# cbs228/sameold

Measured on AMD Instinct MI355X. Metric: Msamples/s demodulated (batched 22.05 kHz channels) + % HBM roofline, 1/8 GPU, higher is better.
Workload: dtype f32

## Files before the change

sameold_amd/csrc/same_batch.cpp:

```cpp
#include <hip/hip_runtime.h>

#include <algorithm>
#include <chrono>
#include <cstdio>
#include <cstdlib>
#include <cstring>
#include <deque>
#include <new>
#include <string>
#include <utility>
#include <vector>

#include "../../include/same_rx.h"
#include "same_config.h"
#include "same_device.h"
#include "same_harvest.h"
#include "same_hipmem.h"
#include "same_launch.h"
#include "same_resets.h"
#include "same_transport.h"

using same::fail;

namespace {
// ... 19 lines not shown
    hipStream_t last_stream = nullptr;
    same::DevBuf<float4> d_taps;
    same::DevBuf<void> d_state_blob;
    struct Slot {
        same::DevBuf<same::DevEvent> d_events;
        uint32_t event_cap() const { return (uint32_t)d_events.size(); }
        same::DevBuf<uint32_t> d_sort;
        same::PinnedBuf<uint32_t> h_sort;
        same::DevBuf<same::DevEvent> d_sorted;
        uint32_t sort_bins = 0;
        same::DevBuf<uint8_t> d_bursts;
        uint32_t burst_cap() const { return (uint32_t)(d_bursts.size() / same::kBurstCap); }
        same::DevBuf<uint32_t> d_counters;
        same::MappedBuf<uint32_t> h_counters;
        same::Event ev_start, ev_stop, ev_done, ev_planned;
        same::Event ev_k0, ev_k1;
        bool have_k = false;
        bool timed = false;
        same::PinnedBuf<void> h_events, h_bursts;
        bool in_flight = false;
        uint64_t seq = 0;
        uint64_t end_counter = 0;
        bool chunked = false;
        same::ChunkGeom geom{};
        uint64_t end_blocks = 0;
        same::DevBuf<uint64_t> d_handover;
        same::PinnedBuf<uint64_t> h_handover;
        bool per_channel = false;
        same::DevBuf<uint32_t> d_geom;
        same::PinnedBuf<uint32_t> h_geom;
        same::CoherentBuf<uint32_t> h_reset;
        same::CoherentBuf<uint32_t> h_counts;
        same::PinnedBuf<uint64_t> h_wake_up;
        bool dev_transport = false;
        same::CoherentBuf<same::DevMessage> h_near;
        uint32_t near_cap() const { return (uint32_t)h_near.size(); }
        same::DevBuf<same::DevMessage> d_msgs;
        uint32_t msg_cap() const { return (uint32_t)d_msgs.size(); }
        same::PinnedBuf<void> h_msgs;
        bool captured = false;
        same::DevBuf<same::cap::Span> d_spans;
        uint32_t span_cap() const { return (uint32_t)d_spans.size(); }
        same::DevBuf<float> d_pool;
        same::DevBuf<same::cap::Cursors> d_cap_cur;
        same::MappedBuf<same::cap::Cursors> h_cap_cur;
        same::PinnedBuf<void> h_spans, h_pool;
    } slot[2];
    struct TimePar {
        bool enabled = false;
        uint32_t max_chunks = 0, min_own = 0, warmup = 0;
        uint32_t cap_columns = 0;
        uint32_t carved_columns = 0;
        int carved_family = -1;
        same::Params Pv{};
        same::State Sv{};
        same::DevBuf<void> blob;
        same::DevBuf<void> blob_fresh;
        size_t fresh_bytes = 0;
        same::DevBuf<same::StateArrayDesc> d_desc_in, d_desc_out;
        uint32_t n_desc = 0;
        same::DevBuf<uint32_t> d_final_col;
        same::DevBuf<float> d_energy;
        same::DevBuf<float> d_hist;
        same::Event ev_plan_prev; bool plan_recorded = false;
        int knob_plan_stream = 0;
        int sort_mode = -1;
        uint32_t last_chunks = 1;
        bool last_per_channel = false;
        same::Family family = same::Family::kPipe;
        int knob_prologue = 0;
    } tp;
    uint64_t launch_seq = 0;
    hipStream_t copy_stream = nullptr;
    struct Windowed {
        bool on = false;
        uint32_t window = 0;
        uint32_t fill = 0;
        same::DevBuf<void> d_buf;
        same::Event ev_buf;
        hipStream_t buf_stream = nullptr; bool buf_used = false;
        same::Event ev_read[2];
        uint64_t n_reads = 0;
        hipStream_t read_stream = nullptr;
    } inv;
    hipStream_t plan_stream = nullptr;
    float last_ms = 0.0f;
    bool overflowed = false;
    std::string record_path;
    bool kernel_fault = false;
    same::Request want;
    same::Mode mode;
    same::Choice plain;
    same::Params Pfm{};
    same::Family last_family = same::Family::kGeneric;
    bool sym_launched = false;
    bool debug = false;
    same::DevBuf<void> d_stage, d_stage2;
    same::DevBuf<void> d_upload;
    same::DevBuf<void> d_zero;
    same::Event ev_order;
    bool timing = false;
    bool have_timing = false;
    float last_demod_ms = 0.0f;
    same::PinnedBuf<uint64_t> h_wake;
    bool wake_ordered = false;
    std::vector<uint32_t> ragged_by;
    bool messages_only = false;
    bool dev_transport = false;
    bool last_dev_transport = false;
    same::DevBuf<void> d_thot, d_tcold;
    same::ResetLedger resets;
    std::vector<uint32_t> reset_list, reset_now, reset_cols;
    same::EventLog events;
    same::Replay replay{resets, events};
    struct Audio {
// ... 79 lines not shown
    rx->P.knob_pipe_split = tri("SAME_PIPE_SPLIT");
#ifdef SAME_PROFILE
    rx->P.knob_mirror = tri("SAME_MIRROR");
    rx->P.knob_pipe_share = tri("SAME_PIPE_SHARE");
    rx->P.knob_prio = num("SAME_PIPE_PRIO", 0);
#endif
    rx->P.knob_fast_dense = tri("SAME_FAST_DENSE");
    rx->P.knob_sym = tri("SAME_SYM");
    rx->want.sym_max_channels = (uint32_t)std::max(0, num("SAME_SYM_MAX", 1 << 30));
    rx->debug = rx->replay.debug = std::getenv("SAME_DEBUG") != nullptr;
    { const char *e = std::getenv("SAME_RECORD_HARVEST"); rx->record_path = e ? e : ""; }
    rx->replay.host_threads = std::max(0, num("SAME_HOST_THREADS", 0));
    rx->tp.sort_mode = num("SAME_TP_SORT", -1);
    rx->tp.knob_plan_stream = tri("SAME_TP_PLAN_STREAM");
    rx->tp.knob_prologue = tri("SAME_TP_PROLOGUE");
    rx->want.knob_relaxed = tri("SAME_RELAXED");
    { const char *e = std::getenv("SAME_RELAXED_KERNEL"); rx->P.knob_relaxed_kernel = !e ? 0 : (std::strcmp(e, "solo") == 0 ? 1 : (std::strcmp(e, "duo") == 0 ? 2 : 0)); }
    { const char *e = std::getenv("SAME_TP_KERNEL"); rx->want.knob_tp_kernel = !e ? 0 : (std::strcmp(e, "wave") == 0 ? 2 : (std::strcmp(e, "pipe") == 0 ? 1 : 0)); }
}

int ensure_output(same_batch *rx, same_batch::Slot &sl, size_t n_samples, same::Output &O, size_t n_columns = 0)
{
    const size_t n_ch = n_columns ? n_columns : rx->P.n_channels;
    const double symbols = (double)n_samples * 520.83 / (double)rx->P.input_rate;
    const size_t per_chan_events = (size_t)(symbols / 8.0) + 16;
    const size_t per_chan_bursts = (size_t)(symbols / 160.0) + 4;
    size_t ecap = std::min<size_t>(per_chan_events * n_ch, 0x7fffffffu / sizeof(same::DevEvent));
    size_t bcap = std::min<size_t>(per_chan_bursts * n_ch, 0x7fffffffu / same::kBurstCap);
    HIP_TRY(sl.d_events.ensure(ecap));
    HIP_TRY(sl.d_bursts.ensure(bcap * same::kBurstCap));
// ... 5 lines not shown
    }
    HIP_TRY(sl.d_sorted.ensure(sl.d_events.size()));
    HIP_TRY(sl.d_sort.ensure(2 * n_ch + 1 + same::event_sort_extra_words((uint32_t)n_ch)));
    HIP_TRY(sl.h_sort.ensure(n_ch + 1));
    sl.sort_bins = (uint32_t)n_ch;
    O.events = sl.d_events; O.event_cap = sl.event_cap();
    O.bursts = sl.d_bursts; O.burst_cap = sl.burst_cap();
    O.n_events = sl.d_counters; O.n_bursts = sl.d_counters + 1; O.overflow = sl.d_counters + 2;
    return SAME_OK;
}

template <typename SampleT>
hipError_t launch_family(same::Family f, const same::Params &P, const same::State &S, const same::Output &O, const float4 *taps, const SampleT *x,
                         uint32_t n_blocks, uint64_t counter0, hipStream_t stream, const same::PipeChunks &pc = same::PipeChunks{})
{
    switch (f) {
    case same::Family::kSym: return same::launch_demod_sym(P, S, O, taps, x, n_blocks, counter0, stream, pc);
    case same::Family::kPipeFastmath: return same::launch_demod_pipe(P, S, O, taps, x, n_blocks, counter0, stream, pc, true);
    case same::Family::kPipe: return same::launch_demod_pipe(P, S, O, taps, x, n_blocks, counter0, stream, pc, false);
    case same::Family::kWaveRelaxed: return same::launch_demod_relaxed(P, S, O, taps, x, n_blocks, counter0, stream, pc);
    case same::Family::kFast: return same::launch_demod_fast(P, S, O, taps, x, n_blocks, counter0, stream);
    case same::Family::kGeneric: break;
    }
    return hipErrorInvalidValue;
}

void reset_channel_host(same_batch *rx, uint32_t c, uint64_t pos)
{
    rx->replay.reset_channel(c, pos);
    if (rx->h_wake) rx->h_wake[c] = 0;
// ... 97 lines not shown
    const int oi = (int)(&other - rx->slot);
    for (uint32_t c = 0; c < C; ++c) {
        const uint64_t w = rx->h_wake[c];
        sl.h_wake_up[c] = w && other.in_flight ? w + rx->resets.pending_shift(oi, c) : w;
    }
    if (other.in_flight) {
        HIP_TRY(hipMemcpyAsync(rx->S.wake_sample, sl.h_wake_up, (size_t)C * sizeof(uint64_t), hipMemcpyHostToDevice, rx->last_stream));
        HIP_TRY(hipEventRecord(other.ev_done, rx->last_stream));
    } else {
        HIP_TRY(hipMemcpyAsync(rx->S.wake_sample, sl.h_wake_up, (size_t)C * sizeof(uint64_t), hipMemcpyHostToDevice, rx->copy_stream));
        HIP_TRY(hipStreamSynchronize(rx->copy_stream));
    }
    return SAME_OK;
}

int harvest_slot(same_batch *rx, same_batch::Slot &sl)
{
    if (!sl.in_flight) return SAME_OK;
    const bool dbg = rx->debug;
    auto t_begin = std::chrono::steady_clock::now();
    HIP_TRY(hipEventSynchronize(sl.ev_done));
    sl.in_flight = false;
    if (sl.timed) {
        HIP_TRY(hipEventElapsedTime(&rx->last_ms, sl.ev_start, sl.ev_stop));
        rx->last_demod_ms = rx->last_ms;
        if (sl.have_k) HIP_TRY(hipEventElapsedTime(&rx->last_demod_ms, sl.ev_k0, sl.ev_k1));
        rx->have_timing = true;
    }
    auto t_waited = std::chrono::steady_clock::now();
    const uint32_t n_events = std::min(sl.h_counters[0], sl.event_cap());
    if (dbg)
        std::fprintf(stderr, "[same] harvest: %u device events (%u bursts), cap %u/%u\n", sl.h_counters[0],
                     sl.h_counters[1], sl.event_cap(), sl.burst_cap());
    const uint32_t n_bursts = std::min(sl.h_counters[1], sl.burst_cap());
    if (sl.h_counters[2] & (3u | same::kMessageLogOverflow)) rx->overflowed = true;
    if (sl.h_counters[2] & 4u) rx->kernel_fault = true;
    if (sl.dev_transport) return harvest_messages(rx, sl, t_begin, t_waited);
    const size_t ev_bytes = (size_t)n_events * sizeof(same::DevEvent), bu_bytes = (size_t)n_bursts * same::kBurstCap;
    HIP_TRY(grow_pinned(sl.h_events, ev_bytes));
    HIP_TRY(grow_pinned(sl.h_bursts, bu_bytes));
    const uint32_t n_ch = rx->P.n_channels;
    const uint32_t n_bins = sl.chunked ? sl.geom.n_chunks * n_ch : n_ch;
    if (n_bins != sl.sort_bins) return fail(SAME_EINVAL, "internal: event sort made for %u columns, launch has %u", sl.sort_bins, n_bins);
    HIP_TRY(hipMemcpyAsync(sl.h_sort, sl.d_sort + n_bins, ((size_t)n_bins + 1) * sizeof(uint32_t), hipMemcpyDeviceToHost, rx->copy_stream));
    if (n_events) HIP_TRY(hipMemcpyAsync(sl.h_events, sl.d_sorted, ev_bytes, hipMemcpyDeviceToHost, rx->copy_stream));
    HIP_TRY(hipStreamSynchronize(rx->copy_stream));
    if (n_bursts) HIP_TRY(hipMemcpyAsync(sl.h_bursts, sl.d_bursts, bu_bytes, hipMemcpyDeviceToHost, rx->copy_stream));
    if (sl.chunked) {
        HIP_TRY(hipMemcpyAsync(sl.h_handover, sl.d_handover, (size_t)n_bins * sizeof(uint64_t), hipMemcpyDeviceToHost, rx->copy_stream));
        if (sl.per_channel)
            HIP_TRY(hipMemcpyAsync(sl.h_geom, sl.d_geom, (size_t)2 * n_bins * sizeof(uint32_t), hipMemcpyDeviceToHost, rx->copy_stream));
    }
    if (n_bursts || sl.chunked) HIP_TRY(hipStreamSynchronize(rx->copy_stream));
    auto t_copied = std::chrono::steady_clock::now();
    const same::HarvestInput in{sl.h_sort, static_cast<same::DevEvent *>(sl.h_events.get()), static_cast<const uint8_t *>(sl.h_bursts.get()),
                                sl.h_handover, sl.h_geom};
    if (!rx->record_path.empty()) { const int rrc = record_harvest(rx, sl, in, n_events, n_bursts, rx->record_path.c_str()); if (rrc != SAME_OK) return rrc; }
    std::vector<uint32_t> rearm;
    same::HarvestTimes times;
    same::HarvestLaunch launch;
    launch.chunked = sl.chunked; launch.per_channel = sl.per_channel; launch.geom = sl.geom;
    launch.end_blocks = sl.end_blocks; launch.end_counter = sl.end_counter;
    int rc = rx->replay.replay(launch, in, n_events, n_bursts, rearm, times);
    if (rc) return rc;
    {
        const int si = (int)(&sl - rx->slot);
        const same::ResetLedger::SlotShift &sh = rx->resets.shift_due(si);
        if (!rx->replay.thot.empty())
            for (size_t i = 0; i < sh.channels.size(); ++i)
// ... 4 lines not shown
        const int si = (int)(&sl - rx->slot);
        const std::vector<uint32_t> &due = rx->resets.host_due(si);
        for (uint32_t c : due) reset_channel_host(rx, c, rx->resets.rec_pos(si));
        rx->resets.done_host(si);
    }
    if (!rearm.empty()) {
        if (!rx->h_wake) {
            HIP_TRY(rx->h_wake.ensure(rx->P.n_channels));
            std::memset(rx->h_wake, 0, (size_t)rx->P.n_channels * sizeof(uint64_t));
        }
        for (uint32_t c : rearm) rx->h_wake[c] = rx->replay.tr(c).force_eom_at();
        if (rx->wake_ordered) {
            int rc2 = upload_wake_ordered(rx, sl);
            if (rc2) return rc2;
        } else {
        HIP_TRY(hipMemcpyAsync(rx->S.wake_sample, rx->h_wake, (size_t)rx->P.n_channels * sizeof(uint64_t), hipMemcpyHostToDevice, rx->copy_stream));
        HIP_TRY(hipStreamSynchronize(rx->copy_stream));
        }
    }
    if (dbg) {
        auto t_end = std::chrono::steady_clock::now();
        auto ms = [](auto a, auto b) { return std::chrono::duration<double, std::milli>(b - a).count(); };
        std::fprintf(stderr, "[same] harvest timing: wait %.2f ms, copy %.2f ms, sort %.2f ms, replay on %u threads %.2f ms, "
                             "queue %.2f ms\n",
                     ms(t_begin, t_waited), ms(t_waited, t_copied), ms(t_copied, times.sorted), times.n_threads,
                     ms(times.sorted, times.replayed), ms(times.replayed, t_end));
    }
    return SAME_OK;
}

int harvest(same_batch *rx)
{
// ... 38 lines not shown
    HIP_TRY(sl.d_handover.ensure(columns));
    HIP_TRY(sl.h_handover.ensure(columns));
    return SAME_OK;
}

int ensure_wide_state(same_batch *rx, uint32_t columns)
{
    same_batch::TimePar &tp = rx->tp;
    if (tp.carved_columns == columns && tp.carved_family == (int)tp.family) return SAME_OK;
    int rc = harvest(rx);
    if (rc) return rc;
    HIP_TRY(hipDeviceSynchronize());
    tp.Pv = same::wide_params(rx->P, columns, same::is_fastmath(tp.family), same::tp_more_than_one_round(columns));
    if (columns > tp.cap_columns) {
        tp.cap_columns = 0;
        HIP_TRY(tp.blob.reset());
        HIP_TRY(tp.blob_fresh.reset());
        const size_t bytes = carve_state(tp.Pv, nullptr, tp.Sv);
        HIP_TRY(tp.blob.ensure(bytes));
        HIP_TRY(hipMemset(tp.blob, 0, bytes));
        HIP_TRY(tp.blob_fresh.ensure(bytes));
        tp.cap_columns = columns;
    }
    const size_t blob_bytes = carve_state(tp.Pv, (char *)tp.blob.get(), tp.Sv);
    {
        same::State Sf{};
        carve_state(tp.Pv, (char *)tp.blob_fresh.get(), Sf);
        HIP_TRY(hipMemset(tp.blob_fresh, 0, blob_bytes));
        HIP_TRY(same::launch_init_state(tp.Pv, Sf, 0, nullptr, 0));
        HIP_TRY(hipDeviceSynchronize());
        tp.fresh_bytes = (size_t)(reinterpret_cast<char *>(tp.Sv.fr_msg) - static_cast<char *>(tp.blob.get()));
    }
    std::vector<same::StateArrayDesc> in, out;
    list_state_arrays(rx->P, rx->S, tp.Sv, in);
    list_state_arrays(rx->P, tp.Sv, rx->S, out);
    tp.n_desc = (uint32_t)in.size();
    HIP_TRY(tp.d_desc_in.ensure(in.size()));
    HIP_TRY(tp.d_desc_out.ensure(out.size()));
    HIP_TRY(tp.d_final_col.ensure(rx->P.n_channels));
    HIP_TRY(hipMemcpy(tp.d_desc_in, in.data(), in.size() * sizeof(same::StateArrayDesc), hipMemcpyHostToDevice));
    HIP_TRY(hipMemcpy(tp.d_desc_out, out.data(), out.size() * sizeof(same::StateArrayDesc), hipMemcpyHostToDevice));
    tp.carved_columns = columns;
    tp.carved_family = (int)tp.family;
    return SAME_OK;
}

struct Ragged {
    const uint32_t *counts = nullptr;
    uint32_t m = 0;
    uint32_t row_off = 0;
};

struct RaggedLaunch {
    uint32_t row0 = 0;
    size_t n_lock = 0;
};


int begin_launch(same_batch *rx, same_batch::Slot &sl, const same_batch::Slot &prev, hipStream_t stream)
{
    int rc = harvest_slot(rx, sl);
    if (rc) return rc;
    if (prev.in_flight && rx->last_stream != stream) HIP_TRY(hipStreamWaitEvent(stream, prev.ev_done, 0));
    return launch_pending_resets(rx, sl, stream);
}

int begin_timing(same_batch *rx, same_batch::Slot &sl, hipStream_t stream)
{
    sl.timed = rx->timing;
    if (sl.timed) HIP_TRY(hipEventRecord(sl.ev_start, stream));
    return SAME_OK;
}

int tp_reserve(same_batch *rx, same_batch::Slot &sl, uint32_t columns, size_t n, const same::PipeChunks &pc, uint32_t block_len, same::Output &O)
{
    int rc = ensure_wide_state(rx, columns);
    if (rc) return rc;
    rc = ensure_output(rx, sl, std::min<size_t>(n, 3 * (size_t)pc.nominal_blocks * block_len + 65536), O, columns);
    if (rc) return rc;
    return ensure_handover(sl, columns);
}

int tp_start(same_batch *rx, same_batch::Slot &sl, uint32_t columns, const char *layout, hipStream_t stream, bool *sort_bins_empty)
{
    same_batch::TimePar &tp = rx->tp;
    const uint32_t C = rx->P.n_channels;
    *sort_bins_empty = false;
    if (tp.knob_prologue >= 0) {
        HIP_TRY(same::launch_tp_prologue(tp.blob, tp.blob_fresh, tp.fresh_bytes, sl.d_handover, sl.d_sort, columns, sl.d_counters, stream));
        *sort_bins_empty = sl.sort_bins == columns;
    } else {
        HIP_TRY(same::launch_counters(sl.d_counters, sl.h_counters.dev(), 0, stream));
        HIP_TRY(same::launch_init_state(tp.Pv, tp.Sv, 0, stream, C));
        HIP_TRY(same::launch_fill_u64(sl.d_handover, columns, same::kNoHandover, stream));
    }
    if (rx->debug) std::fprintf(stderr, "[same] time-parallel launch: %u columns (%s), start-up: %s\n", columns, layout,
                                tp.knob_prologue >= 0 ? "prologue kernel" : "separate launches");
    HIP_TRY(same::launch_copy_state_columns(tp.d_desc_in, tp.n_desc, C, columns, nullptr, C, stream));
    return SAME_OK;
}

int tp_hand_back(same_batch *rx, same_batch::Slot &sl, const same::ChunkGeom &geom, const uint32_t *own_start, hipStream_t stream)
{
    same_batch::TimePar &tp = rx->tp;
    const uint32_t C = rx->P.n_channels;
    if (own_start) HIP_TRY(same::launch_chunk_final_column_pc(sl.d_handover, own_start, C, geom.n_chunks, rx->counter, tp.d_final_col, stream));
    else HIP_TRY(same::launch_chunk_final_column(sl.d_handover, C, geom, tp.d_final_col, stream));
    HIP_TRY(same::launch_copy_state_columns(tp.d_desc_out, tp.n_desc, geom.n_chunks * C, C, tp.d_final_col, C, stream));
    return SAME_OK;
}

template <typename SampleT>
int demod_tail(same_batch *rx, const same::Output &O, const SampleT *rows, size_t n, uint64_t counter0, hipStream_t stream)
{
    const hipError_t e = same::launch_demod(rx->P, rx->S, O, rx->d_taps, rows, (uint32_t)n, counter0, stream);
    if (e != hipSuccess) return fail(SAME_EHIP, "demod kernel launch failed: %s", hipGetErrorString(e));
    return SAME_OK;
}
int demod_tail_corner(same_batch *rx, const same::Output &O, const float *corner, size_t pitch, size_t r, uint64_t counter0, hipStream_t stream)
{
    const uint32_t C = rx->P.n_channels;
    HIP_TRY(rx->d_stage.ensure(r * C * sizeof(float)));
    HIP_TRY(rx->d_stage2.ensure(r * C * sizeof(float)));
// ... 80 lines not shown
        bool sort_bins_empty = false;
        same::Output O{};
        if (n_chunks > 1u) {
            const uint32_t C = rx->P.n_channels, columns = n_chunks * C;
            const size_t fbk = geom.block_len;
            rc = tp_reserve(rx, sl, columns, n, pc, geom.block_len, O);
            if (rc) return rc;
            pc.handover = sl.d_handover;
            same_batch::TimePar &tp = rx->tp;
            rc = begin_timing(rx, sl, stream);
            if (rc) return rc;
            rc = tp_start(rx, sl, columns, "time-major", stream, &sort_bins_empty);
            if (rc) return rc;
            const SampleT *xp = d_x + done * C;
            const uint32_t total_blocks = (uint32_t)(n / fbk);
            const hipError_t e = launch_family(tp.family, tp.Pv, tp.Sv, O, rx->d_taps, xp, total_blocks, rx->counter, stream, pc);
            rx->last_family = tp.family;
            if (e != hipSuccess) return fail(SAME_EHIP, "time-parallel demod kernel launch failed: %s", hipGetErrorString(e));
            rc = tp_hand_back(rx, sl, geom, nullptr, stream);
            if (rc) return rc;
            const size_t n_whole = (size_t)total_blocks * fbk;
            if (n_whole < n && (rc = demod_tail(rx, O, xp + n_whole * C, n - n_whole, rx->counter + n_whole, stream)) != SAME_OK) return rc;
            sl.chunked = true; sl.per_channel = false;
            sl.geom = geom;
            sl.end_blocks = rx->counter + n_whole;
            rx->tp.last_per_channel = false;
        } else {
        sl.chunked = false; sl.per_channel = false;
        rc = ensure_output(rx, sl, n, O);
        if (rc) return rc;
        HIP_TRY(same::launch_counters(sl.d_counters, sl.h_counters.dev(), 0, stream));
// ... 158 lines not shown
        const uint32_t warm = tp.warmup ? tp.warmup : (uint32_t)(40.0 * sps + 0.5);
        plan.warmup_samples = std::min(geom.warmup_blocks, (warm + fb - 1u) / fb) * fb;
    }
    plan.whole_samples = (uint32_t)n; plan.in_samples = n_call;
    plan.scout_blocks = (uint32_t)(n / same::tp_scout_block());
    HIP_TRY(tp.d_energy.ensure((size_t)C * plan.scout_blocks));
    uint32_t *d_own = sl.d_geom, *d_row0 = sl.d_geom + columns, *d_nom = sl.d_geom + 2 * (size_t)columns,
             *d_perm = sl.d_geom + 3 * (size_t)columns, *d_wg = sl.d_geom + 4 * (size_t)columns,
             *d_wg2 = d_wg + columns / same::kWave, *d_perm2 = d_wg2 + 2 * (columns / same::kWave);
    const bool pair_groups = tp.sort_mode == 2 && tp.family == same::Family::kSym;
    const int sort_mode = pair_groups ? 0 : (tp.sort_mode >= 0 ? (tp.sort_mode ? 1 : 0) : (same::tp_more_than_one_round(columns) ? 1 : 0));
    rc = begin_timing(rx, sl, stream);
    if (rc) return rc;
    const bool lpt = sort_mode != 0 || pair_groups;
    const bool side = stream == rx->own_stream && tp.knob_plan_stream >= 0;
    hipStream_t ps = side ? rx->plan_stream : stream;
    if (tp.plan_recorded) HIP_TRY(hipStreamWaitEvent(ps, tp.ev_plan_prev, 0));
    HIP_TRY(same::launch_tp_plan(d_x, plan, tp.d_energy, d_own, d_row0, d_nom, d_perm, d_wg, sort_mode != 0, ps,
                                 lpt ? d_perm2 : nullptr, lpt ? d_wg2 : nullptr, pair_groups));
    HIP_TRY(tp.ev_plan_prev.ensure());
    HIP_TRY(hipEventRecord(tp.ev_plan_prev, ps));
    tp.plan_recorded = true;
    if (side) {
        HIP_TRY(hipEventRecord(sl.ev_planned, ps));
        HIP_TRY(hipStreamWaitEvent(stream, sl.ev_planned, 0));
    }
    if (lpt) { d_perm = d_perm2; d_wg = d_wg2; }
    bool sort_bins_empty = false;
    rc = tp_start(rx, sl, columns, "channel-major", stream, &sort_bins_empty);
    if (rc) return rc;
    pc.handover = sl.d_handover;
    pc.col_row0 = d_row0; pc.col_nominal = d_nom; pc.wg_blocks = d_wg; pc.col_perm = (sort_mode != 0 || pair_groups) ? d_perm : nullptr;
    pc.in_samples = n_call; pc.whole_samples = (uint32_t)n;
    pc.hist_scratch = nullptr;
    if (pc.col_perm && tp.family == same::Family::kSym) {
        HIP_TRY(tp.d_hist.ensure((size_t)columns * same::kSquelchHist));
        pc.hist_scratch = tp.d_hist;
    }
    sl.have_k = sl.timed;
    if (sl.timed) HIP_TRY(hipEventRecord(sl.ev_k0, stream));
    const hipError_t e = launch_family(tp.family, tp.Pv, tp.Sv, O, rx->d_taps, d_x, (uint32_t)(n / fb), rx->counter, stream, pc);
    rx->last_family = tp.family;
    if (e != hipSuccess) return fail(SAME_EHIP, "time-parallel demod kernel launch failed: %s", hipGetErrorString(e));
    if (sl.timed) HIP_TRY(hipEventRecord(sl.ev_k1, stream));
    rc = tp_hand_back(rx, sl, geom, d_own, stream);
    if (rc) return rc;
    if (n < n_call && (rc = demod_tail_corner(rx, O, d_x + n, n_call, n_call - n, rx->counter + n, stream)) != SAME_OK) return rc;
    sl.chunked = true; sl.per_channel = true;
    sl.geom = geom;
    sl.end_blocks = rx->counter + n;
    tp.last_chunks = n_chunks; tp.last_per_channel = true;
    rc = end_launch<float>(rx, sl, prev, stream, nullptr, n_call, sort_bins_empty);
    return rc ? rc : 1;
}
int process_channel_major_native(same_batch *, const int16_t *, size_t, hipStream_t) { return 0; }

template <typename SampleT, typename Launch>
int transpose_in_slabs(same_batch *rx, const SampleT *d_x, size_t pitch, size_t n_rows, hipStream_t stream, Launch &&launch)
{
    const uint32_t C = rx->P.n_channels;
    for (same_batch::Slot &sl : rx->slot)
        if (sl.in_flight && rx->last_stream != stream) HIP_TRY(hipStreamWaitEvent(stream, sl.ev_done, 0));
    const size_t slab = std::min<size_t>(n_rows, (size_t)65520);
    HIP_TRY(rx->d_stage2.ensure(slab * C * sizeof(SampleT)));
// ... 209 lines not shown
    rx->Pfm = same::fm_params(rx->P);
    rx->last_family = same::strict_family(rx->P, rx->mode);
    if (same::demod_lds_bytes(rx->P) > 160 * 1024)
        return cleanup(fail(SAME_EINVAL, "configuration needs %zu bytes of LDS per wavefront (limit 160 KiB)", same::demod_lds_bytes(rx->P)));
    TRY_OR_CLEAN(hipStreamCreateWithFlags(&rx->own_stream, hipStreamNonBlocking));
    TRY_OR_CLEAN(hipStreamCreateWithFlags(&rx->copy_stream, hipStreamNonBlocking));
    TRY_OR_CLEAN(hipStreamCreateWithFlags(&rx->plan_stream, hipStreamNonBlocking));
    TRY_OR_CLEAN(rx->ev_order.ensure());
    for (auto &sl : rx->slot) {
        TRY_OR_CLEAN(sl.ev_start.ensure(hipEventDefault));
        TRY_OR_CLEAN(sl.ev_stop.ensure(hipEventDefault));
        TRY_OR_CLEAN(sl.ev_k0.ensure(hipEventDefault));
        TRY_OR_CLEAN(sl.ev_k1.ensure(hipEventDefault));
        TRY_OR_CLEAN(sl.ev_done.ensure());
        TRY_OR_CLEAN(sl.ev_planned.ensure());
        TRY_OR_CLEAN(sl.d_counters.ensure(4));
        TRY_OR_CLEAN(sl.h_counters.ensure(4));
    }
    static_assert(sizeof(float4) == 4 * sizeof(float), "the taps are uploaded in fours");
    TRY_OR_CLEAN(rx->d_taps.ensure(taps.size() / 4));
    TRY_OR_CLEAN(hipMemcpy(rx->d_taps, taps.data(), taps.size() * sizeof(float), hipMemcpyHostToDevice));
    const size_t state_bytes = carve_state(rx->P, nullptr, rx->S);
    TRY_OR_CLEAN(rx->d_state_blob.ensure(state_bytes));
    TRY_OR_CLEAN(hipMemset(rx->d_state_blob, 0, state_bytes));
    carve_state(rx->P, (char *)rx->d_state_blob.get(), rx->S);
    TRY_OR_CLEAN(same::launch_init_state(rx->P, rx->S, 0, rx->own_stream));
    if (rx->dev_transport) {
        TRY_OR_CLEAN(rx->d_thot.ensure((size_t)n_channels * same::transport_hot_bytes()));
        TRY_OR_CLEAN(rx->d_tcold.ensure((size_t)n_channels * same::transport_cold_bytes()));
        TRY_OR_CLEAN(hipMemsetAsync(rx->d_tcold, 0, (size_t)n_channels * same::transport_cold_bytes(), rx->own_stream));
// ... 127 lines not shown
{
    if (!rx) return fail(SAME_EINVAL, "null handle");
    if (!rx->inv.on) return fail(SAME_EINVAL, "the batch was not made with SAME_BATCH_CALL_INVARIANT");
    if (samples < 64u || samples > (1u << 22)) return fail(SAME_EINVAL, "window of %u samples (64 .. 4 194 304)", samples);
    if (rx->counter || rx->inv.fill) return fail(SAME_EINVAL, "the window is set before the first sample (or right behind a reset)");
    rx->inv.window = samples;
    return SAME_OK;
}

int same_batch_order_after(same_batch *rx, void *producer_stream)
{
    if (!rx) return fail(SAME_EINVAL, "null handle");
    if (producer_stream == SAME_STREAM_OWN) return SAME_OK;
    HIP_TRY(hipSetDevice(rx->device));
    HIP_TRY(hipEventRecord(rx->ev_order, (hipStream_t)producer_stream));
    HIP_TRY(hipStreamWaitEvent(rx->own_stream, rx->ev_order, 0));
    HIP_TRY(hipStreamWaitEvent(rx->plan_stream, rx->ev_order, 0));
    return SAME_OK;
}

int same_batch_sync(same_batch *rx)
{
    if (!rx) return fail(SAME_EINVAL, "null handle");
    HIP_TRY(hipSetDevice(rx->device));
    int rc = harvest(rx);
    if (rc == SAME_OK && rx->inv.on) rc = inv_reads_wait(rx);
    if (rc) return rc;
    if (rx->kernel_fault) return fail(SAME_EKERNEL, "a demodulation kernel's wavefronts lost step (internal hand-over timed out)");
    if (rx->overflowed) return fail(SAME_EOVERFLOW, "event/burst pool overflow");
    return SAME_OK;
// ... 280 lines not shown
```

sameold_amd/csrc/same_device.h:

```cpp
#pragma once

#include <stddef.h>
#include <stdint.h>

namespace same {

constexpr int kWave = 64;
constexpr int kMaxEqTaps = 16;
constexpr int kBurstCap = 288;
constexpr int kSquelchHist = 64;
constexpr int kMaxTaps = 512;

struct Params {
    uint32_t n_channels;
    uint32_t input_rate;
    uint32_t dc_len;
    float dc_inv_len;
    float dc_k;
    float agc_bw, agc_min, agc_max, agc_gain0;
    uint32_t ntaps;
    uint32_t win_ring;
    float samples_per_ted, period_min, period_max;
    float alpha_unlocked, beta_unlocked, alpha_locked, beta_locked;
    uint32_t sync_word, sq_max_errors;
// ... 70 lines not shown
};

struct PipeChunks {
    uint32_t n_chunks;
    uint32_t in_channels;
    uint32_t stride_blocks;
    uint32_t nominal_blocks;
    uint64_t *handover;
    const uint32_t *col_row0;
    const uint32_t *col_nominal;
    const uint32_t *wg_blocks;
    const uint32_t *col_perm;
    float *hist_scratch;
    uint64_t in_samples;
    uint32_t whole_samples;
};

struct ChunkGeom {
    uint64_t counter0;
    uint32_t n_chunks, block_len, stride_blocks, warmup_blocks;
#if defined(__HIPCC__)
    __host__ __device__
#endif
    uint32_t owner_of(uint64_t h) const
    {
        const uint64_t blocks = (h - counter0) / block_len;
        if (blocks < warmup_blocks) return 0u;
        const uint64_t k = (blocks - warmup_blocks) / stride_blocks;
        return k >= n_chunks ? n_chunks - 1u : (uint32_t)k;
    }
// ... 43 lines not shown
```

sameold_amd/csrc/same_kernels_sym.hip:

```cpp
#include <hip/hip_runtime.h>

#include <cmath>
#include <cstdlib>
#include <mutex>
#include <set>
#include <type_traits>
#include <utility>

#include "same_dev_common.h"
#include "same_device.h"
#include "same_fast_common.h"
#include "same_launch.h"
#include "same_pipe_common.h"
#include "same_profile.h"
#include "same_relaxed_common.h"

namespace same {

constexpr int kSymSub = 36;
constexpr uint32_t kSymDrain = 5u;
constexpr uint32_t kSymOffMask = 255u;
template <int NT> struct SymGeom;
template <> struct SymGeom<42> { static constexpr int DCL = 16, NSUB = 1, HALVES = 2; };
template <> struct SymGeom<92> { static constexpr int DCL = 35, NSUB = 2, HALVES = 1; };
// ... 887 lines not shown
    const uint32_t wave = (uint32_t)__builtin_amdgcn_readfirstlane((int)(threadIdx.x >> 6));
    constexpr uint64_t kDeal0 = 0xdcba98543210ull;
#ifdef SAME_PROFILE
    const uint32_t deal = ((uint32_t)P.knob_prio >> 14) & 3u;
    constexpr uint64_t kDeal1 = 0x805d192ab3c4ull;
    constexpr uint64_t kDeal2 = 0x08d591a2b3c4ull;
    constexpr uint64_t kDeal3 = 0x2ad51908b3c4ull;
    const uint64_t tbl = deal == 0u ? kDeal0 : (deal == 1u ? kDeal1 : (deal == 2u ? kDeal2 : kDeal3));
#else
    constexpr uint64_t tbl = kDeal0;
#endif
    const uint32_t hr = LY::HALVES == 2 ? (uint32_t)(tbl >> (4u * wave)) & 15u : wave;
    const uint32_t half = LY::HALVES == 2 ? hr >> 3 : 0u;
    const uint32_t role = hr & 7u;
    const uint32_t C = P.n_channels;
    const uint32_t vwg = blockIdx.x * kSymHalves + half;
    if (vwg * kWave >= C) return;
    float *lds = lds_all + half * (uint32_t)(LY::lds_bytes / sizeof(float));
    const uint32_t c = (K.n_chunks > 1u && K.col_perm) ? K.col_perm[vwg * kWave + lane] : vwg * kWave + lane;
    uint32_t cin = c, Cin = C, n_nominal = n_blocks;
    bool may_leave = false;
    int32_t row_l = 0;
    const SampleT *xl = nullptr;
    uint32_t avail_l = 0;
    if (K.n_chunks > 1u) {
        Cin = K.in_channels;
        if (K.col_row0) {
            const uint32_t chunk_l = c / Cin;
            cin = c - chunk_l * Cin;
            may_leave = (uint32_t)__builtin_amdgcn_readfirstlane((int)chunk_l) + 1u < K.n_chunks;
            const uint32_t row_abs = K.col_row0[c];
            xl = x + (size_t)cin * K.in_samples + row_abs;
// ... 724 lines not shown
    if (n_blocks == 0u) return hipSuccess;
    auto go = [&](auto kernel) -> hipError_t {
        if (lds > 64u * 1024u) {
            static std::mutex mu;
            static std::set<std::pair<const void *, int>> opted_in;
            int dev = 0;
            if (hipGetDevice(&dev) != hipSuccess) return hipErrorInvalidDevice;
            const std::pair<const void *, int> key(reinterpret_cast<const void *>(kernel), dev);
            std::lock_guard<std::mutex> lock(mu);
            if (opted_in.find(key) == opted_in.end()) {
                const hipError_t e = hipFuncSetAttribute(key.first, hipFuncAttributeMaxDynamicSharedMemorySize, (int)lds);
                if (e != hipSuccess) return e;
                opted_in.insert(key);
            }
        }
        hipLaunchKernelGGL(kernel, dim3((P.n_channels / kWave + kSymHalves - 1u) / kSymHalves), dim3(kSymHalves * kSymRoles * kWave), lds, stream, P, S, O, taps, x, n_blocks, counter0, K);
        return hipGetLastError();
    };
    if constexpr (std::is_same<SampleT, float>::value && NT == 42) {
        if (cm) return go(demod_sym_kernel<NT, NFF, NFB, float, 1>);
    }
    return go(demod_sym_kernel<NT, NFF, NFB, SampleT, 0>);
}

template <typename SampleT>
static hipError_t launch_sym_hi_t(const Params &P, const State &S, const Output &O, const float4 *taps, const SampleT *x,
                                  uint32_t n_blocks, uint64_t counter0, hipStream_t stream, const PipeChunks &K)
{
    const bool eq = P.eq_nff == 6u && P.eq_nfb == 4u;
    if (standard_rate_taps(P) == 92u)
        return eq ? launch_sym_one<92, 6, 4, SampleT>(P, S, O, taps, x, n_blocks, counter0, stream, K) : launch_sym_one<92, 1, 1, SampleT>(P, S, O, taps, x, n_blocks, counter0, stream, K);
// ... 47 lines not shown
```

Baseline: 466,800.

## Split time-parallel sym launch so fresh pieces overlap previous launch

The time-parallel symbol demod launch is split in two when the plan runs on a side stream. The columns that start from fresh state (every piece after the first) are launched on a per-slot side stream right after the prologue, so they can run alongside the previous launch. Only the first piece, which needs the carried-over channel state, waits on the main stream for the state copy-in. Per-slot state blobs and descriptors are double-buffered so the two slots do not share scratch state, at the cost of extra memory, more streams and events, and more complex ordering.

```diff
diff --git a/sameold_amd/csrc/same_batch.cpp b/sameold_amd/csrc/same_batch.cpp
--- a/sameold_amd/csrc/same_batch.cpp
+++ b/sameold_amd/csrc/same_batch.cpp
@@ -57,6 +57,8 @@
         same::DevBuf<uint32_t> d_counters;
         same::MappedBuf<uint32_t> h_counters;
         same::Event ev_start, ev_stop, ev_done, ev_planned;
+        same::Event ev_prologue, ev_body;
+        bool overlapped = false;
         same::Event ev_k0, ev_k1;
         bool have_k = false;
         bool timed = false;
@@ -72,6 +74,8 @@
         bool per_channel = false;
         same::DevBuf<uint32_t> d_geom;
         same::PinnedBuf<uint32_t> h_geom;
+        const uint32_t *d_wg = nullptr;
+        bool grid_order = false;
         same::CoherentBuf<uint32_t> h_reset;
         same::CoherentBuf<uint32_t> h_counts;
         same::PinnedBuf<uint64_t> h_wake_up;
@@ -96,11 +100,11 @@
         uint32_t carved_columns = 0;
         int carved_family = -1;
         same::Params Pv{};
-        same::State Sv{};
-        same::DevBuf<void> blob;
+        same::State Sv[2]{};
+        same::DevBuf<void> blob[2];
         same::DevBuf<void> blob_fresh;
         size_t fresh_bytes = 0;
-        same::DevBuf<same::StateArrayDesc> d_desc_in, d_desc_out;
+        same::DevBuf<same::StateArrayDesc> d_desc_in[2], d_desc_out[2];
         uint32_t n_desc = 0;
         same::DevBuf<uint32_t> d_final_col;
         same::DevBuf<float> d_energy;
@@ -112,6 +116,7 @@
         bool last_per_channel = false;
         same::Family family = same::Family::kPipe;
         int knob_prologue = 0;
+        int knob_overlap = 0;
     } tp;
     uint64_t launch_seq = 0;
     hipStream_t copy_stream = nullptr;
@@ -142,6 +147,7 @@
     same::DevBuf<void> d_upload;
     same::DevBuf<void> d_zero;
     same::Event ev_order;
+    bool order_recorded = false;
     bool timing = false;
     bool have_timing = false;
     float last_demod_ms = 0.0f;
@@ -251,6 +257,7 @@
     rx->tp.sort_mode = num("SAME_TP_SORT", -1);
     rx->tp.knob_plan_stream = tri("SAME_TP_PLAN_STREAM");
     rx->tp.knob_prologue = tri("SAME_TP_PROLOGUE");
+    rx->tp.knob_overlap = tri("SAME_TP_OVERLAP");
     rx->want.knob_relaxed = tri("SAME_RELAXED");
     { const char *e = std::getenv("SAME_RELAXED_KERNEL"); rx->P.knob_relaxed_kernel = !e ? 0 : (std::strcmp(e, "solo") == 0 ? 1 : (std::strcmp(e, "duo") == 0 ? 2 : 0)); }
     { const char *e = std::getenv("SAME_TP_KERNEL"); rx->want.knob_tp_kernel = !e ? 0 : (std::strcmp(e, "wave") == 0 ? 2 : (std::strcmp(e, "pipe") == 0 ? 1 : 0)); }
@@ -286,6 +293,7 @@
 hipError_t launch_family(same::Family f, const same::Params &P, const same::State &S, const same::Output &O, const float4 *taps, const SampleT *x,
                          uint32_t n_blocks, uint64_t counter0, hipStream_t stream, const same::PipeChunks &pc = same::PipeChunks{})
 {
+    if (pc.n_groups && f != same::Family::kSym) return hipErrorInvalidValue;
     switch (f) {
     case same::Family::kSym: return same::launch_demod_sym(P, S, O, taps, x, n_blocks, counter0, stream, pc);
     case same::Family::kPipeFastmath: return same::launch_demod_pipe(P, S, O, taps, x, n_blocks, counter0, stream, pc, true);
@@ -413,10 +421,51 @@
     return SAME_OK;
 }
 
+hipStream_t slot_stream(same_batch *rx, const same_batch::Slot &sl) { return &sl == &rx->slot[0] ? rx->copy_stream : rx->plan_stream; }
+
+int debug_occupancy(same_batch *rx, same_batch::Slot &sl)
+{
+    hipStream_t cs = sl.overlapped ? slot_stream(rx, sl) : rx->copy_stream;
+    const uint32_t C = rx->P.n_channels, columns = sl.geom.n_chunks * C, groups = columns / same::kWave, fb = sl.geom.block_len;
+    const uint32_t whole = (uint32_t)(sl.end_blocks - sl.geom.counter0);
+    std::vector<uint32_t> wg(groups), nominal(columns), plan(groups, 0u);
+    HIP_TRY(hipMemcpyAsync(wg.data(), sl.d_wg, (size_t)groups * sizeof(uint32_t), hipMemcpyDeviceToHost, cs));
+    HIP_TRY(hipMemcpyAsync(nominal.data(), sl.d_geom + 2 * (size_t)columns, (size_t)columns * sizeof(uint32_t), hipMemcpyDeviceToHost, cs));
+    HIP_TRY(hipStreamSynchronize(cs));
+    if (sl.grid_order)
+        for (uint32_t v = 0; v < columns; ++v) {
+            const uint32_t avail = (whole - sl.h_geom[columns + v]) / fb;
+            plan[v / same::kWave] = std::max(plan[v / same::kWave], v / C + 1u == sl.geom.n_chunks ? avail : std::min(nominal[v], avail));
+        }
+    const uint32_t n_wg = (groups + 1u) / 2u, per = C / same::kWave;
+    auto report = [&](const char *what, const std::vector<uint32_t> &len) {
+        double sum = 0.0; uint32_t longest = 0;
+        for (uint32_t g = 0; g < groups; g += 2u) {
+            const uint32_t m = std::max(len[g], g + 1u < groups ? len[g + 1u] : 0u);
+            sum += m; longest = std::max(longest, m);
+        }
+        std::fprintf(stderr, "[same] occupancy (%s): %u workgroups, steps mean %.1f max %u, rho %.4f", what, n_wg, sum / n_wg, longest,
+                     longest ? sum / n_wg / longest : 0.0);
+        if (sl.grid_order) {
+            std::fprintf(stderr, "; by piece, mean / max of its groups:");
+            for (uint32_t k = 0; k < sl.geom.n_chunks; ++k) {
+                double s = 0.0; uint32_t mx = 0;
+                for (uint32_t g = 0; g < per; ++g) { s += len[k * per + g]; mx = std::max(mx, len[k * per + g]); }
+                std::fprintf(stderr, " %.0f/%u", s / per, mx);
+            }
+        }
+        std::fprintf(stderr, "\n");
+    };
+    report("wg_blocks", wg);
+    if (sl.grid_order) report("planned", plan);
+    return SAME_OK;
+}
+
 int harvest_slot(same_batch *rx, same_batch::Slot &sl)
 {
     if (!sl.in_flight) return SAME_OK;
     const bool dbg = rx->debug;
+    hipStream_t cs = sl.overlapped ? slot_stream(rx, sl) : rx->copy_stream;
     auto t_begin = std::chrono::steady_clock::now();
     HIP_TRY(hipEventSynchronize(sl.ev_done));
     sl.in_flight = false;
@@ -425,6 +474,9 @@
         rx->last_demod_ms = rx->last_ms;
         if (sl.have_k) HIP_TRY(hipEventElapsedTime(&rx->last_demod_ms, sl.ev_k0, sl.ev_k1));
         rx->have_timing = true;
+        float lead = 0.0f;
+        if (dbg && sl.overlapped && hipEventElapsedTime(&lead, sl.ev_prologue, sl.ev_start) == hipSuccess)
+            std::fprintf(stderr, "[same] two launches: the body was free to begin %.3f ms before the launch stream reached this launch\n", lead);
     }
     auto t_waited = std::chrono::steady_clock::now();
     const uint32_t n_events = std::min(sl.h_counters[0], sl.event_cap());
@@ -441,17 +493,18 @@
     const uint32_t n_ch = rx->P.n_channels;
     const uint32_t n_bins = sl.chunked ? sl.geom.n_chunks * n_ch : n_ch;
     if (n_bins != sl.sort_bins) return fail(SAME_EINVAL, "internal: event sort made for %u columns, launch has %u", sl.sort_bins, n_bins);
-    HIP_TRY(hipMemcpyAsync(sl.h_sort, sl.d_sort + n_bins, ((size_t)n_bins + 1) * sizeof(uint32_t), hipMemcpyDeviceToHost, rx->copy_stream));
-    if (n_events) HIP_TRY(hipMemcpyAsync(sl.h_events, sl.d_sorted, ev_bytes, hipMemcpyDeviceToHost, rx->copy_stream));
-    HIP_TRY(hipStreamSynchronize(rx->copy_stream));
-    if (n_bursts) HIP_TRY(hipMemcpyAsync(sl.h_bursts, sl.d_bursts, bu_bytes, hipMemcpyDeviceToHost, rx->copy_stream));
+    HIP_TRY(hipMemcpyAsync(sl.h_sort, sl.d_sort + n_bins, ((size_t)n_bins + 1) * sizeof(uint32_t), hipMemcpyDeviceToHost, cs));
+    if (n_events) HIP_TRY(hipMemcpyAsync(sl.h_events, sl.d_sorted, ev_bytes, hipMemcpyDeviceToHost, cs));
+    HIP_TRY(hipStreamSynchronize(cs));
+    if (n_bursts) HIP_TRY(hipMemcpyAsync(sl.h_bursts, sl.d_bursts, bu_bytes, hipMemcpyDeviceToHost, cs));
     if (sl.chunked) {
-        HIP_TRY(hipMemcpyAsync(sl.h_handover, sl.d_handover, (size_t)n_bins * sizeof(uint64_t), hipMemcpyDeviceToHost, rx->copy_stream));
+        HIP_TRY(hipMemcpyAsync(sl.h_handover, sl.d_handover, (size_t)n_bins * sizeof(uint64_t), hipMemcpyDeviceToHost, cs));
         if (sl.per_channel)
-            HIP_TRY(hipMemcpyAsync(sl.h_geom, sl.d_geom, (size_t)2 * n_bins * sizeof(uint32_t), hipMemcpyDeviceToHost, rx->copy_stream));
-    }
-    if (n_bursts || sl.chunked) HIP_TRY(hipStreamSynchronize(rx->copy_stream));
+            HIP_TRY(hipMemcpyAsync(sl.h_geom, sl.d_geom, (size_t)2 * n_bins * sizeof(uint32_t), hipMemcpyDeviceToHost, cs));
+    }
+    if (n_bursts || sl.chunked) HIP_TRY(hipStreamSynchronize(cs));
     auto t_copied = std::chrono::steady_clock::now();
+    if (dbg && sl.chunked && sl.per_channel && sl.d_wg) { const int orc = debug_occupancy(rx, sl); if (orc) return orc; }
     const same::HarvestInput in{sl.h_sort, static_cast<same::DevEvent *>(sl.h_events.get()), static_cast<const uint8_t *>(sl.h_bursts.get()),
                                 sl.h_handover, sl.h_geom};
     if (!rx->record_path.empty()) { const int rrc = record_harvest(rx, sl, in, n_events, n_bursts, rx->record_path.c_str()); if (rrc != SAME_OK) return rrc; }
@@ -486,8 +539,8 @@
             int rc2 = upload_wake_ordered(rx, sl);
             if (rc2) return rc2;
         } else {
-        HIP_TRY(hipMemcpyAsync(rx->S.wake_sample, rx->h_wake, (size_t)rx->P.n_channels * sizeof(uint64_t), hipMemcpyHostToDevice, rx->copy_stream));
-        HIP_TRY(hipStreamSynchronize(rx->copy_stream));
+        HIP_TRY(hipMemcpyAsync(rx->S.wake_sample, rx->h_wake, (size_t)rx->P.n_channels * sizeof(uint64_t), hipMemcpyHostToDevice, cs));
+        HIP_TRY(hipStreamSynchronize(cs));
         }
     }
     if (dbg) {
@@ -556,32 +609,37 @@
     tp.Pv = same::wide_params(rx->P, columns, same::is_fastmath(tp.family), same::tp_more_than_one_round(columns));
     if (columns > tp.cap_columns) {
         tp.cap_columns = 0;
-        HIP_TRY(tp.blob.reset());
+        for (auto &b : tp.blob) HIP_TRY(b.reset());
         HIP_TRY(tp.blob_fresh.reset());
-        const size_t bytes = carve_state(tp.Pv, nullptr, tp.Sv);
-        HIP_TRY(tp.blob.ensure(bytes));
-        HIP_TRY(hipMemset(tp.blob, 0, bytes));
+        const size_t bytes = carve_state(tp.Pv, nullptr, tp.Sv[0]);
+        for (auto &b : tp.blob) {
+            HIP_TRY(b.ensure(bytes));
+            HIP_TRY(hipMemset(b, 0, bytes));
+        }
         HIP_TRY(tp.blob_fresh.ensure(bytes));
         tp.cap_columns = columns;
     }
-    const size_t blob_bytes = carve_state(tp.Pv, (char *)tp.blob.get(), tp.Sv);
+    size_t blob_bytes = 0;
+    for (int s = 0; s < 2; ++s) blob_bytes = carve_state(tp.Pv, (char *)tp.blob[s].get(), tp.Sv[s]);
     {
         same::State Sf{};
         carve_state(tp.Pv, (char *)tp.blob_fresh.get(), Sf);
         HIP_TRY(hipMemset(tp.blob_fresh, 0, blob_bytes));
         HIP_TRY(same::launch_init_state(tp.Pv, Sf, 0, nullptr, 0));
         HIP_TRY(hipDeviceSynchronize());
-        tp.fresh_bytes = (size_t)(reinterpret_cast<char *>(tp.Sv.fr_msg) - static_cast<char *>(tp.blob.get()));
-    }
-    std::vector<same::StateArrayDesc> in, out;
-    list_state_arrays(rx->P, rx->S, tp.Sv, in);
-    list_state_arrays(rx->P, tp.Sv, rx->S, out);
-    tp.n_desc = (uint32_t)in.size();
-    HIP_TRY(tp.d_desc_in.ensure(in.size()));
-    HIP_TRY(tp.d_desc_out.ensure(out.size()));
+        tp.fresh_bytes = (size_t)(reinterpret_cast<char *>(tp.Sv[0].fr_msg) - static_cast<char *>(tp.blob[0].get()));
+    }
     HIP_TRY(tp.d_final_col.ensure(rx->P.n_channels));
-    HIP_TRY(hipMemcpy(tp.d_desc_in, in.data(), in.size() * sizeof(same::StateArrayDesc), hipMemcpyHostToDevice));
-    HIP_TRY(hipMemcpy(tp.d_desc_out, out.data(), out.size() * sizeof(same::StateArrayDesc), hipMemcpyHostToDevice));
+    for (int s = 0; s < 2; ++s) {
+        std::vector<same::StateArrayDesc> in, out;
+        list_state_arrays(rx->P, rx->S, tp.Sv[s], in);
+        list_state_arrays(rx->P, tp.Sv[s], rx->S, out);
+        tp.n_desc = (uint32_t)in.size();
+        HIP_TRY(tp.d_desc_in[s].ensure(in.size()));
+        HIP_TRY(tp.d_desc_out[s].ensure(out.size()));
+        HIP_TRY(hipMemcpy(tp.d_desc_in[s], in.data(), in.size() * sizeof(same::StateArrayDesc), hipMemcpyHostToDevice));
+        HIP_TRY(hipMemcpy(tp.d_desc_out[s], out.data(), out.size() * sizeof(same::StateArrayDesc), hipMemcpyHostToDevice));
+    }
     tp.carved_columns = columns;
     tp.carved_family = (int)tp.family;
     return SAME_OK;
@@ -603,6 +661,7 @@
 {
     int rc = harvest_slot(rx, sl);
     if (rc) return rc;
+    sl.overlapped = false;
     if (prev.in_flight && rx->last_stream != stream) HIP_TRY(hipStreamWaitEvent(stream, prev.ev_done, 0));
     return launch_pending_resets(rx, sl, stream);
 }
@@ -623,23 +682,35 @@
     return ensure_handover(sl, columns);
 }
 
-int tp_start(same_batch *rx, same_batch::Slot &sl, uint32_t columns, const char *layout, hipStream_t stream, bool *sort_bins_empty)
+int tp_fresh_columns(same_batch *rx, same_batch::Slot &sl, uint32_t columns, const char *layout, hipStream_t stream, bool *sort_bins_empty)
 {
     same_batch::TimePar &tp = rx->tp;
     const uint32_t C = rx->P.n_channels;
+    const int si = (int)(&sl - rx->slot);
     *sort_bins_empty = false;
     if (tp.knob_prologue >= 0) {
-        HIP_TRY(same::launch_tp_prologue(tp.blob, tp.blob_fresh, tp.fresh_bytes, sl.d_handover, sl.d_sort, columns, sl.d_counters, stream));
+        HIP_TRY(same::launch_tp_prologue(tp.blob[si], tp.blob_fresh, tp.fresh_bytes, sl.d_handover, sl.d_sort, columns, sl.d_counters, stream));
         *sort_bins_empty = sl.sort_bins == columns;
     } else {
         HIP_TRY(same::launch_counters(sl.d_counters, sl.h_counters.dev(), 0, stream));
-        HIP_TRY(same::launch_init_state(tp.Pv, tp.Sv, 0, stream, C));
+        HIP_TRY(same::launch_init_state(tp.Pv, tp.Sv[si], 0, stream, C));
         HIP_TRY(same::launch_fill_u64(sl.d_handover, columns, same::kNoHandover, stream));
     }
     if (rx->debug) std::fprintf(stderr, "[same] time-parallel launch: %u columns (%s), start-up: %s\n", columns, layout,
                                 tp.knob_prologue >= 0 ? "prologue kernel" : "separate launches");
-    HIP_TRY(same::launch_copy_state_columns(tp.d_desc_in, tp.n_desc, C, columns, nullptr, C, stream));
-    return SAME_OK;
+    return SAME_OK;
+}
+int tp_own_state_in(same_batch *rx, same_batch::Slot &sl, uint32_t columns, hipStream_t stream)
+{
+    same_batch::TimePar &tp = rx->tp;
+    const uint32_t C = rx->P.n_channels;
+    HIP_TRY(same::launch_copy_state_columns(tp.d_desc_in[&sl - rx->slot], tp.n_desc, C, columns, nullptr, C, stream));
+    return SAME_OK;
+}
+int tp_start(same_batch *rx, same_batch::Slot &sl, uint32_t columns, const char *layout, hipStream_t stream, bool *sort_bins_empty)
+{
+    const int rc = tp_fresh_columns(rx, sl, columns, layout, stream, sort_bins_empty);
+    return rc ? rc : tp_own_state_in(rx, sl, columns, stream);
 }
 
 int tp_hand_back(same_batch *rx, same_batch::Slot &sl, const same::ChunkGeom &geom, const uint32_t *own_start, hipStream_t stream)
@@ -648,7 +719,7 @@
     const uint32_t C = rx->P.n_channels;
     if (own_start) HIP_TRY(same::launch_chunk_final_column_pc(sl.d_handover, own_start, C, geom.n_chunks, rx->counter, tp.d_final_col, stream));
     else HIP_TRY(same::launch_chunk_final_column(sl.d_handover, C, geom, tp.d_final_col, stream));
-    HIP_TRY(same::launch_copy_state_columns(tp.d_desc_out, tp.n_desc, geom.n_chunks * C, C, tp.d_final_col, C, stream));
+    HIP_TRY(same::launch_copy_state_columns(tp.d_desc_out[&sl - rx->slot], tp.n_desc, geom.n_chunks * C, C, tp.d_final_col, C, stream));
     return SAME_OK;
 }
 
@@ -759,7 +830,7 @@
             if (rc) return rc;
             const SampleT *xp = d_x + done * C;
             const uint32_t total_blocks = (uint32_t)(n / fbk);
-            const hipError_t e = launch_family(tp.family, tp.Pv, tp.Sv, O, rx->d_taps, xp, total_blocks, rx->counter, stream, pc);
+            const hipError_t e = launch_family(tp.family, tp.Pv, tp.Sv[&sl - rx->slot], O, rx->d_taps, xp, total_blocks, rx->counter, stream, pc);
             rx->last_family = tp.family;
             if (e != hipSuccess) return fail(SAME_EHIP, "time-parallel demod kernel launch failed: %s", hipGetErrorString(e));
             rc = tp_hand_back(rx, sl, geom, nullptr, stream);
@@ -948,21 +1019,31 @@
     if (rc) return rc;
     const bool lpt = sort_mode != 0 || pair_groups;
     const bool side = stream == rx->own_stream && tp.knob_plan_stream >= 0;
-    hipStream_t ps = side ? rx->plan_stream : stream;
+    const bool overlap = side && tp.knob_overlap >= 0 && tp.knob_prologue >= 0 && tp.family == same::Family::kSym && !lpt;
+    hipStream_t bs = slot_stream(rx, sl);
+    hipStream_t ps = overlap ? bs : (side ? rx->plan_stream : stream);
+    sl.overlapped = overlap;
     if (tp.plan_recorded) HIP_TRY(hipStreamWaitEvent(ps, tp.ev_plan_prev, 0));
+    if (overlap && rx->order_recorded) HIP_TRY(hipStreamWaitEvent(ps, rx->ev_order, 0));
     HIP_TRY(same::launch_tp_plan(d_x, plan, tp.d_energy, d_own, d_row0, d_nom, d_perm, d_wg, sort_mode != 0, ps,
                                  lpt ? d_perm2 : nullptr, lpt ? d_wg2 : nullptr, pair_groups));
     HIP_TRY(tp.ev_plan_prev.ensure());
     HIP_TRY(hipEventRecord(tp.ev_plan_prev, ps));
     tp.plan_recorded = true;
-    if (side) {
+    if (side && !overlap) {
         HIP_TRY(hipEventRecord(sl.ev_planned, ps));
         HIP_TRY(hipStreamWaitEvent(stream, sl.ev_planned, 0));
     }
     if (lpt) { d_perm = d_perm2; d_wg = d_wg2; }
     bool sort_bins_empty = false;
-    rc = tp_start(rx, sl, columns, "channel-major", stream, &sort_bins_empty);
-    if (rc) return rc;
+    if (overlap) {
+        rc = tp_fresh_columns(rx, sl, columns, "channel-major, its fresh pieces beside the previous launch", bs, &sort_bins_empty);
+        if (rc) return rc;
+        HIP_TRY(hipEventRecord(sl.ev_prologue, bs));
+    } else {
+        rc = tp_start(rx, sl, columns, "channel-major", stream, &sort_bins_empty);
+        if (rc) return rc;
+    }
     pc.handover = sl.d_handover;
     pc.col_row0 = d_row0; pc.col_nominal = d_nom; pc.wg_blocks = d_wg; pc.col_perm = (sort_mode != 0 || pair_groups) ? d_perm : nullptr;
     pc.in_samples = n_call; pc.whole_samples = (uint32_t)n;
@@ -972,8 +1053,25 @@
         pc.hist_scratch = tp.d_hist;
     }
     sl.have_k = sl.timed;
-    if (sl.timed) HIP_TRY(hipEventRecord(sl.ev_k0, stream));
-    const hipError_t e = launch_family(tp.family, tp.Pv, tp.Sv, O, rx->d_taps, d_x, (uint32_t)(n / fb), rx->counter, stream, pc);
+    const same::State &Sv = tp.Sv[&sl - rx->slot];
+    hipError_t e = hipSuccess;
+    if (overlap) {
+        const uint32_t head_groups = C / same::kWave;
+        pc.first_group = head_groups; pc.n_groups = columns / same::kWave - head_groups;
+        e = launch_family(tp.family, tp.Pv, Sv, O, rx->d_taps, d_x, (uint32_t)(n / fb), rx->counter, bs, pc);
+        if (e != hipSuccess) return fail(SAME_EHIP, "time-parallel demod kernel launch failed: %s", hipGetErrorString(e));
+        HIP_TRY(hipEventRecord(sl.ev_body, bs));
+        HIP_TRY(hipStreamWaitEvent(stream, sl.ev_prologue, 0));
+        rc = tp_own_state_in(rx, sl, columns, stream);
+        if (rc) return rc;
+        if (sl.timed) HIP_TRY(hipEventRecord(sl.ev_k0, stream));
+        pc.first_group = 0u; pc.n_groups = head_groups;
+        e = launch_family(tp.family, tp.Pv, Sv, O, rx->d_taps, d_x, (uint32_t)(n / fb), rx->counter, stream, pc);
+        if (e == hipSuccess) HIP_TRY(hipStreamWaitEvent(stream, sl.ev_body, 0));
+    } else {
+        if (sl.timed) HIP_TRY(hipEventRecord(sl.ev_k0, stream));
+        e = launch_family(tp.family, tp.Pv, Sv, O, rx->d_taps, d_x, (uint32_t)(n / fb), rx->counter, stream, pc);
+    }
     rx->last_family = tp.family;
     if (e != hipSuccess) return fail(SAME_EHIP, "time-parallel demod kernel launch failed: %s", hipGetErrorString(e));
     if (sl.timed) HIP_TRY(hipEventRecord(sl.ev_k1, stream));
@@ -982,6 +1080,7 @@
     if (n < n_call && (rc = demod_tail_corner(rx, O, d_x + n, n_call, n_call - n, rx->counter + n, stream)) != SAME_OK) return rc;
     sl.chunked = true; sl.per_channel = true;
     sl.geom = geom;
+    sl.d_wg = d_wg; sl.grid_order = pc.col_perm == nullptr;
     sl.end_blocks = rx->counter + n;
     tp.last_chunks = n_chunks; tp.last_per_channel = true;
     rc = end_launch<float>(rx, sl, prev, stream, nullptr, n_call, sort_bins_empty);
@@ -1221,6 +1320,8 @@
         TRY_OR_CLEAN(sl.ev_k1.ensure(hipEventDefault));
         TRY_OR_CLEAN(sl.ev_done.ensure());
         TRY_OR_CLEAN(sl.ev_planned.ensure());
+        TRY_OR_CLEAN(sl.ev_prologue.ensure(hipEventDefault));
+        TRY_OR_CLEAN(sl.ev_body.ensure());
         TRY_OR_CLEAN(sl.d_counters.ensure(4));
         TRY_OR_CLEAN(sl.h_counters.ensure(4));
     }
@@ -1378,6 +1479,7 @@
     if (producer_stream == SAME_STREAM_OWN) return SAME_OK;
     HIP_TRY(hipSetDevice(rx->device));
     HIP_TRY(hipEventRecord(rx->ev_order, (hipStream_t)producer_stream));
+    rx->order_recorded = true;
     HIP_TRY(hipStreamWaitEvent(rx->own_stream, rx->ev_order, 0));
     HIP_TRY(hipStreamWaitEvent(rx->plan_stream, rx->ev_order, 0));
     return SAME_OK;
diff --git a/sameold_amd/csrc/same_device.h b/sameold_amd/csrc/same_device.h
--- a/sameold_amd/csrc/same_device.h
+++ b/sameold_amd/csrc/same_device.h
@@ -108,6 +108,7 @@
     float *hist_scratch;
     uint64_t in_samples;
     uint32_t whole_samples;
+    uint32_t first_group, n_groups;
 };
 
 struct ChunkGeom {
diff --git a/sameold_amd/csrc/same_kernels_sym.hip b/sameold_amd/csrc/same_kernels_sym.hip
--- a/sameold_amd/csrc/same_kernels_sym.hip
+++ b/sameold_amd/csrc/same_kernels_sym.hip
@@ -925,8 +925,8 @@
     const uint32_t half = LY::HALVES == 2 ? hr >> 3 : 0u;
     const uint32_t role = hr & 7u;
     const uint32_t C = P.n_channels;
-    const uint32_t vwg = blockIdx.x * kSymHalves + half;
-    if (vwg * kWave >= C) return;
+    const uint32_t vwg = K.first_group + blockIdx.x * kSymHalves + half;
+    if (vwg >= (K.n_groups ? K.first_group + K.n_groups : C / kWave)) return;
     float *lds = lds_all + half * (uint32_t)(LY::lds_bytes / sizeof(float));
     const uint32_t c = (K.n_chunks > 1u && K.col_perm) ? K.col_perm[vwg * kWave + lane] : vwg * kWave + lane;
     uint32_t cin = c, Cin = C, n_nominal = n_blocks;
@@ -1681,7 +1681,8 @@
                 opted_in.insert(key);
             }
         }
-        hipLaunchKernelGGL(kernel, dim3((P.n_channels / kWave + kSymHalves - 1u) / kSymHalves), dim3(kSymHalves * kSymRoles * kWave), lds, stream, P, S, O, taps, x, n_blocks, counter0, K);
+        const uint32_t groups = K.n_groups ? K.n_groups : P.n_channels / kWave;
+        hipLaunchKernelGGL(kernel, dim3((groups + kSymHalves - 1u) / kSymHalves), dim3(kSymHalves * kSymRoles * kWave), lds, stream, P, S, O, taps, x, n_blocks, counter0, K);
         return hipGetLastError();
     };
     if constexpr (std::is_same<SampleT, float>::value && NT == 42) {
```

Result: faster. 485,000 (median of 5 runs) (+3.9%).
